# iiscleap/NeuralPlda

Measured on AMD Instinct MI355X. Metric: scored trial-pairs/sec (512-d xvec), higher is better.
Workload: dtype f32; 1 GPU; cfg1: 1048576 trial pairs/GPU/step, 512->150->150 NPLDA, scoring only (fused NeuralPlda.forward, inputs resident in HBM); xvector_dim=512, layer1_LDA_dim=150, layer2_PLDA_spkfactor_dim=150, params=kaldi-init truncated to 150, parallelism=trial-list shard x1, backend=single process, ranks_in_group=1

## Files before the change

### neuralplda_amd/csrc/nplda_fwd_dispatch.h

```cpp
#pragma once
#include <cstdlib>
#include <cstring>
#include "nplda_fwd_kernel.h"
#include "nplda_fwd_small.h"
#include "nplda_fwd_v2.h"
#include "nplda_fwd_v3.h"
#include "nplda_fwd_v5.h"
#include "nplda_fwd_v6.h"
#include "nplda_fwd_mid.h"

namespace nplda {

template <int MODE>
static inline int launch_fwd_v2(FwdArgs a, const NpldaLayout& L, hipStream_t st) {
    constexpr int WAVES = 8;
    const long long per_block = (MODE == MODE_EMBED ? 32 : 16) * WAVES;
    const long long blocks = (a.n + per_block - 1) / per_block;
    if (blocks > 0x7fffffffLL) return NPLDA_EINVAL;
    dim3 grid((unsigned)blocks), block(WAVES * 64);
#define NPLDA_LAUNCH(NBV) \
    hipLaunchKernelGGL((nplda_fwd_v2_kernel<NBV, MODE, WAVES, false, (NBV == 2 ? 4 : 2)>), grid, block, 0, st, a)
    switch (L.NB) {
        case 2: NPLDA_LAUNCH(2); break;
        case 4: NPLDA_LAUNCH(4); break;
        case 8: NPLDA_LAUNCH(8); break;
        case 10: NPLDA_LAUNCH(10); break;
        case 11: NPLDA_LAUNCH(11); break;
        case 12: NPLDA_LAUNCH(12); break;
        default: return NPLDA_EUNSUPPORTED;
    }
#undef NPLDA_LAUNCH
    return nplda_launch_status();
}

template <int MODE, int XM = 0>
static inline int launch_fwd_v3(FwdArgs a, const NpldaLayout& L, hipStream_t st) {
    constexpr int WAVES = 8;
    const long long per_block = (MODE == MODE_EMBED ? 32 : 16) * WAVES;
    const long long ntiles = (a.n + per_block - 1) / per_block;
    if (ntiles > 0x7fffffffLL) return NPLDA_EINVAL;
    int dev = 0, cus = 0;
    if (hipGetDevice(&dev) != hipSuccess ||
        hipDeviceGetAttribute(&cus, hipDeviceAttributeMultiprocessorCount, dev) != hipSuccess || cus <= 0)
        cus = 256;
    const long long blocks = ntiles < cus ? ntiles : cus;
    dim3 grid((unsigned)blocks), block(WAVES * 64);
#define NPLDA_LAUNCH(NBV) \
    hipLaunchKernelGGL((nplda_fwd_v3_kernel<NBV, MODE, WAVES, XM, (NBV == 2 ? 4 : 2)>), grid, block, 0, st, a, (int)ntiles)
    switch (L.NB) {
        case 2: NPLDA_LAUNCH(2); break;
        case 4: NPLDA_LAUNCH(4); break;
        case 8: NPLDA_LAUNCH(8); break;
        case 10: NPLDA_LAUNCH(10); break;
        default: return NPLDA_EUNSUPPORTED;
    }
#undef NPLDA_LAUNCH
    return nplda_launch_status();
}

template <int XM = 0>
static inline int launch_fwd_v5(FwdArgs a, const NpldaLayout& L, hipStream_t st) {
    constexpr int WAVES = 8;
    const long long ntiles = (a.n + 16 * WAVES - 1) / (16 * WAVES);
    if (ntiles > 0x7fffffffLL) return NPLDA_EINVAL;
    int dev = 0, cus = 0;
    if (hipGetDevice(&dev) != hipSuccess ||
        hipDeviceGetAttribute(&cus, hipDeviceAttributeMultiprocessorCount, dev) != hipSuccess || cus <= 0)
        cus = 256;
    const long long blocks = ntiles < cus ? ntiles : cus;
    dim3 grid((unsigned)blocks), block(WAVES * 64);
    switch (L.NB) {
        case 11: hipLaunchKernelGGL((nplda_fwd_v5_kernel<11, WAVES, 2, 6, 1, XM>), grid, block, 0, st, a, (int)ntiles); break;
        case 12: hipLaunchKernelGGL((nplda_fwd_v5_kernel<12, WAVES, 4, 4, 1, XM>), grid, block, 0, st, a, (int)ntiles); break;
        default: return NPLDA_EUNSUPPORTED;
    }
    return nplda_launch_status();
}

static inline bool fwd_v6_ok(const NpldaLayout& L) { return L.NB == 10 && L.D1 == 150 && L.D2 == 150; }
static inline bool fwd_v6_l2_f32() {
    static const bool f32 = getenv("NPLDA_FWD_V6_L2") != nullptr && strcmp(getenv("NPLDA_FWD_V6_L2"), "f32") == 0;
    return f32;
}
template <int XM = 0>
static inline int launch_fwd_v6(FwdArgs a, const NpldaLayout& L, hipStream_t st) {
    constexpr int WAVES = 8;
    const long long ntiles = (a.n + 16 * WAVES - 1) / (16 * WAVES);
    if (ntiles > 0x7fffffffLL) return NPLDA_EINVAL;
    if (!fwd_v6_ok(L)) return NPLDA_EUNSUPPORTED;
    int dev = 0, cus = 0;
    if (hipGetDevice(&dev) != hipSuccess ||
        hipDeviceGetAttribute(&cus, hipDeviceAttributeMultiprocessorCount, dev) != hipSuccess || cus <= 0)
        cus = 256;
    const long long blocks = ntiles < cus ? ntiles : cus;
    if (fwd_v6_l2_f32())
        hipLaunchKernelGGL((nplda_fwd_v6_kernel<10, 6, WAVES, 2, 5, 3, XM, 0, 2, 0>), dim3((unsigned)blocks), dim3(WAVES * 64), 0, st, a,
                           (int)ntiles);
    else
        hipLaunchKernelGGL((nplda_fwd_v6_kernel<10, 6, WAVES, 2, 5, 3, XM, 0, 2, 1>), dim3((unsigned)blocks), dim3(WAVES * 64), 0, st, a,
                           (int)ntiles);
    return nplda_launch_status();
}
template <int XM = 0>
static inline int launch_fwd_stream(FwdArgs a, const NpldaLayout& L, hipStream_t st) {
    static const bool no_v6 = getenv("NPLDA_FWD_NO_V6") != nullptr && getenv("NPLDA_FWD_NO_V6")[0] == '1';
    if (fwd_v6_ok(L) && !no_v6) return launch_fwd_v6<XM>(a, L, st);
    if (L.NB <= 10) return launch_fwd_v3<MODE_PAIR, XM>(a, L, st);
    return launch_fwd_v5<XM>(a, L, st);
}

template <int MODE>
static inline int launch_fwd_small(FwdArgs a, const NpldaLayout& L, hipStream_t st) {
    const long long per_block = (MODE == MODE_EMBED ? 32 : 16);
    const long long blocks = (a.n + per_block - 1) / per_block;
    dim3 grid((unsigned)blocks), block(256);
#define NPLDA_LAUNCH(NBV) hipLaunchKernelGGL((nplda_fwd_small_kernel<NBV, MODE>), grid, block, 0, st, a)
#define NPLDA_LAUNCH32(NBV)                                                                           \
    if (L.KS1 == 32 && L.D0 == 512) hipLaunchKernelGGL((nplda_fwd_small_kernel<NBV, MODE, 32>), grid, block, 0, st, a); \
    else NPLDA_LAUNCH(NBV)
    switch (L.NB) {
        case 2: NPLDA_LAUNCH(2); break;
        case 4: NPLDA_LAUNCH(4); break;
        case 8: NPLDA_LAUNCH(8); break;
        case 10: NPLDA_LAUNCH32(10); break;
        case 11: NPLDA_LAUNCH32(11); break;
        case 12: NPLDA_LAUNCH(12); break;
        default: return NPLDA_EUNSUPPORTED;
    }
#undef NPLDA_LAUNCH32
#undef NPLDA_LAUNCH
    return nplda_launch_status();
}

static inline int mid_cus() {
    int dev = 0, cus = 0;
    if (hipGetDevice(&dev) != hipSuccess ||
        hipDeviceGetAttribute(&cus, hipDeviceAttributeMultiprocessorCount, dev) != hipSuccess || cus <= 0)
        cus = 256;
    return cus;
}
template <bool EMBED = false>
static inline int launch_fwd_mid(FwdArgs a, const NpldaLayout& L, hipStream_t st) {
    const long long nh = EMBED ? (a.n + 15) / 16 : (a.n + 7) / 8;
    const int cus = mid_cus();
    long long grid = nh <= cus ? nh : ((nh + 1) / 2 < cus ? (nh + 1) / 2 : cus);
    if (grid < 1) grid = 1;
    const long long c = (nh + grid - 1) / grid;
    const long long r = nh - grid * (c - 1);
    if (c > 0x7fffffffLL) return NPLDA_EINVAL;
    const bool half = !(r == grid && (c & 1) == 0);
    const bool idx = a.ia != nullptr;
#define NPLDA_LAUNCH(NBV, HV, IV) \
    hipLaunchKernelGGL((nplda_fwd_mid_kernel<NBV, EMBED, HV, IV>), dim3((unsigned)grid), dim3(256), 0, st, a, (int)c, (int)r)
#define NPLDA_LAUNCH_H(NBV, HV) do { if (idx) { NPLDA_LAUNCH(NBV, HV, true); } else { NPLDA_LAUNCH(NBV, HV, false); } } while (0)
    switch (L.NB) {
        case 10: if (half) NPLDA_LAUNCH_H(10, true); else NPLDA_LAUNCH_H(10, false); break;
        case 11: if (half) NPLDA_LAUNCH_H(11, true); else NPLDA_LAUNCH_H(11, false); break;
        default: return NPLDA_EUNSUPPORTED;
    }
#undef NPLDA_LAUNCH_H
#undef NPLDA_LAUNCH
    return nplda_launch_status();
}

template <int MODE>
static inline int launch_fwd_old(FwdArgs a, const NpldaLayout& L, hipStream_t st) {
    a.D0 = L.D0; a.KS1 = L.KS1;
    a.oW2 = L.oW2; a.ob1 = L.ob1; a.ob2 = L.ob2; a.oQ = L.oQ; a.oP = L.oP; a.total = L.total;
    const long long units = (MODE == MODE_EMBED ? (a.n + 1) / 2 : a.n);
    if (units <= 256 * 64) return launch_fwd_small<MODE>(a, L, st);
    if constexpr (MODE == MODE_PAIR) return launch_fwd_stream<0>(a, L, st);
    return launch_fwd_v2<MODE>(a, L, st);
}

enum { FWD_SMALL = 0, FWD_MID = 1, FWD_STREAM = 2, FWD_SPLIT = 3 };
static inline long long pair_split_point(long long n, int cus) { return (n / 128 / cus) * 128 * cus; }
static inline int pair_kernel_choice(long long n, const NpldaLayout& L, int cus, long long* cost = nullptr, bool allow_split = true) {
    long long dummy;
    if (!cost) cost = &dummy;
    static const bool no_mid = getenv("NPLDA_FWD_NO_MID") != nullptr && getenv("NPLDA_FWD_NO_MID")[0] == '1';
    const bool mid_ok = !no_mid && (L.NB == 10 || L.NB == 11) && L.D0 == 512 && L.KS1 == 32;
    static const long long small_max = getenv("NPLDA_FWD_SMALL_MAX") ? atoll(getenv("NPLDA_FWD_SMALL_MAX")) : -1;
    const long long round_cost = L.NB == 10 ? 1000 : 1150;
    *cost = 120;
    if (mid_ok && small_max < 0 && n <= 8LL * cus) return FWD_MID;
    *cost = 190;
    if (n <= (small_max >= 0 ? small_max : 16LL * cus)) return FWD_SMALL;
    const long long rounds = ((n + 127) / 128 + cus - 1) / cus;
    const long long t_stream = 50 + rounds * round_cost;
    *cost = n <= 64LL * cus ? 190 * ((n + 16LL * cus - 1) / (16LL * cus)) : t_stream;
    if (!mid_ok) return n <= 64LL * cus ? FWD_SMALL : FWD_STREAM;
    const long long ch = ((n + 7) / 8 + cus - 1) / cus;
    const long long t_mid = 40 + (ch / 2) * (L.NB == 10 ? 133 : 168) + (ch & 1) * (L.NB == 10 ? 93 : 118);
    int best = t_mid < t_stream ? FWD_MID : FWD_STREAM;
    *cost = t_mid < t_stream ? t_mid : t_stream;
    static const bool no_split = getenv("NPLDA_FWD_NO_SPLIT") != nullptr && getenv("NPLDA_FWD_NO_SPLIT")[0] == '1';
    const long long full = pair_split_point(n, cus);
    if (allow_split && !no_split && full > 0 && full < n) {
        long long t_rem = 0;
        pair_kernel_choice(n - full, L, cus, &t_rem, false);
        const long long t_split = 50 + (full / 128 / cus) * round_cost + t_rem;
        if (t_split + 30 < *cost) {
            *cost = t_split;
            best = FWD_SPLIT;
        }
    }
    return best;
}

template <int MODE>
static inline int launch_fwd(FwdArgs a, const NpldaLayout& L, hipStream_t st) {
    if constexpr (MODE == MODE_PAIR) {
        const int cus = mid_cus();
        const int k = pair_kernel_choice(a.n, L, cus);
        a.D0 = L.D0; a.KS1 = L.KS1;
        a.oW2 = L.oW2; a.ob1 = L.ob1; a.ob2 = L.ob2; a.oQ = L.oQ; a.oP = L.oP; a.total = L.total;
        if (k == FWD_MID) return launch_fwd_mid<false>(a, L, st);
        if (k == FWD_SMALL) return launch_fwd_small<MODE>(a, L, st);
        if (k == FWD_SPLIT && a.ia == nullptr && a.ib == nullptr) {
            const long long full = pair_split_point(a.n, cus);
            FwdArgs b = a;
            b.xa += full * a.ldx; b.xb += full * a.ldx; b.out_s += full; b.n = a.n - full;
            a.n = full;
            if (int rc = launch_fwd_stream<0>(a, L, st)) return rc;
            const int kr = pair_kernel_choice(b.n, L, cus, nullptr, false);
            if (kr == FWD_MID) return launch_fwd_mid<false>(b, L, st);
            if (kr == FWD_SMALL) return launch_fwd_small<MODE>(b, L, st);
            return launch_fwd_stream<0>(b, L, st);
        }
        return launch_fwd_stream<0>(a, L, st);
    }
    if constexpr (MODE == MODE_EMBED) {
        if (a.out_y == nullptr && pair_kernel_choice((a.n + 1) / 2, L, mid_cus(), nullptr, false) == FWD_MID) {
            a.D0 = L.D0; a.KS1 = L.KS1;
            a.oW2 = L.oW2; a.ob1 = L.ob1; a.ob2 = L.ob2; a.oQ = L.oQ; a.oP = L.oP; a.total = L.total;
            return launch_fwd_mid<true>(a, L, st);
        }
    }
    return launch_fwd_old<MODE>(a, L, st);
}

static inline int launch_fwd_pairs_bf16rows(FwdArgs a, const NpldaLayout& L, hipStream_t st) {
    const int k = pair_kernel_choice(a.n, L, mid_cus());
    if (k != FWD_STREAM && k != FWD_SPLIT) return NPLDA_EUNSUPPORTED;
    a.D0 = L.D0; a.KS1 = L.KS1;
    a.oW2 = L.oW2; a.ob1 = L.ob1; a.ob2 = L.ob2; a.oQ = L.oQ; a.oP = L.oP; a.total = L.total;
    return launch_fwd_stream<2>(a, L, st);
}

static inline const char* pair_kernel_name(long long n, const NpldaLayout& L) {
    switch (pair_kernel_choice(n, L, mid_cus())) {
        case FWD_SPLIT:
            return pair_kernel_name(pair_split_point(n, mid_cus()), L);
        case FWD_SMALL: return "nplda_fwd_small_kernel (4 waves share a 16-pair tile, feature-split)";
        case FWD_MID: return "nplda_fwd_mid_kernel (balanced 16-pair tiles, K-split layer 1, groups of 2 tiles)";
        default:
            if (fwd_v6_ok(L) && !(getenv("NPLDA_FWD_NO_V6") != nullptr && getenv("NPLDA_FWD_NO_V6")[0] == '1'))
                return fwd_v6_l2_f32()
                           ? "nplda_fwd_v6_kernel (persistent, 9 feature blocks on 16x16x4 MFMAs + 6 features on 4x4x1 MFMAs)"
                           : "nplda_fwd_v6_kernel (persistent, layer 1: 9 feature blocks on 16x16x4 MFMAs + 6 features on 4x4x1 "
                             "MFMAs; layer 2: split bf16x3, 6 passes of 16x16x32)";
            return L.NB <= 10 ? "nplda_fwd_v3_kernel (persistent, 8 waves x 16 pairs, weights through LDS)"
                              : "nplda_fwd_v5_kernel (persistent, LDS-DMA weight chunks, layer 2 by output groups)";
    }
}

static inline int check_model(int D0, int D1, int D2) {
    if (D0 <= 0 || D1 <= 0 || D2 <= 0 || (D0 % 4) != 0) return NPLDA_EINVAL;
    if (!nplda_dims_ok(D0, D1, D2)) return NPLDA_EUNSUPPORTED;
    return NPLDA_OK;
}

static inline bool rows_ok(const float* x, int64_t ld, int D) {
    return x && ld >= D && (ld % 4) == 0 && nplda_aligned16(x);
}

}
```

Baseline: 366.2 million pairs/s.

## Add hybrid v6h kernel running part of layer 1 on split-bf16x3 MFMAs

Adds a new persistent kernel in which layer 1 computes some 16-wide feature blocks with fp32 16x16x4 MFMAs and S1 blocks with weights and inputs split into three bf16 parts, using 16x16x32 bf16 MFMAs. The split W1 blocks are converted by register staging into LDS alongside the existing DMA path. This replaces the old 4x4x1 MFMA handling of the leftover features. Dispatch uses it by default with S1=3, selectable through environment variables. The aim is to move more layer-1 work onto higher-throughput bf16 MFMAs while keeping near-fp32 accuracy, at the cost of extra split ALU work, more LDS, and register pressure.

After: 383.4 million pairs/s (median of 6 runs). 1.05x the previous value.

```diff
diff --git a/neuralplda_amd/csrc/nplda_fwd_dispatch.h b/neuralplda_amd/csrc/nplda_fwd_dispatch.h
--- a/neuralplda_amd/csrc/nplda_fwd_dispatch.h
+++ b/neuralplda_amd/csrc/nplda_fwd_dispatch.h
@@ -7,6 +7,7 @@
 #include "nplda_fwd_v3.h"
 #include "nplda_fwd_v5.h"
 #include "nplda_fwd_v6.h"
+#include "nplda_fwd_v6h.h"
 #include "nplda_fwd_mid.h"
 
 namespace nplda {
@@ -82,6 +83,22 @@
     static const bool f32 = getenv("NPLDA_FWD_V6_L2") != nullptr && strcmp(getenv("NPLDA_FWD_V6_L2"), "f32") == 0;
     return f32;
 }
+enum { FWD_V6H_S1_DEFAULT = 3 };
+static inline bool fwd_v6h_s1_built(int s1) { return s1 == 2 || s1 == 3 || s1 == 4; }
+static inline int fwd_v6h_s1_env() {
+    static const int s1 = [] {
+        const char* f = getenv("NPLDA_FWD_V6_L1");
+        if (f != nullptr && strcmp(f, "f32") == 0) return 0;
+        const char* n = getenv("NPLDA_FWD_V6_L1S");
+        if (n != nullptr && fwd_v6h_s1_built(atoi(n))) return atoi(n);
+        return (int)FWD_V6H_S1_DEFAULT;
+    }();
+    return s1;
+}
+static inline int fwd_v6h_s1(const NpldaLayout& L) {
+    if (!fwd_v6_ok(L) || fwd_v6_l2_f32() || (L.KS1 & 1) != 0) return 0;
+    return fwd_v6h_s1_env();
+}
 template <int XM = 0>
 static inline int launch_fwd_v6(FwdArgs a, const NpldaLayout& L, hipStream_t st) {
     constexpr int WAVES = 8;
@@ -93,12 +110,17 @@
         hipDeviceGetAttribute(&cus, hipDeviceAttributeMultiprocessorCount, dev) != hipSuccess || cus <= 0)
         cus = 256;
     const long long blocks = ntiles < cus ? ntiles : cus;
-    if (fwd_v6_l2_f32())
-        hipLaunchKernelGGL((nplda_fwd_v6_kernel<10, 6, WAVES, 2, 5, 3, XM, 0, 2, 0>), dim3((unsigned)blocks), dim3(WAVES * 64), 0, st, a,
-                           (int)ntiles);
-    else
-        hipLaunchKernelGGL((nplda_fwd_v6_kernel<10, 6, WAVES, 2, 5, 3, XM, 0, 2, 1>), dim3((unsigned)blocks), dim3(WAVES * 64), 0, st, a,
-                           (int)ntiles);
+    const dim3 grid((unsigned)blocks), block(WAVES * 64);
+    switch (fwd_v6h_s1(L)) {
+        case 2: hipLaunchKernelGGL((nplda_fwd_v6h_kernel<10, WAVES, 2, 4, XM>), grid, block, 0, st, a, (int)ntiles); break;
+        case 3: hipLaunchKernelGGL((nplda_fwd_v6h_kernel<10, WAVES, 3, 4, XM>), grid, block, 0, st, a, (int)ntiles); break;
+        case 4: hipLaunchKernelGGL((nplda_fwd_v6h_kernel<10, WAVES, 4, 3, XM>), grid, block, 0, st, a, (int)ntiles); break;
+        default:
+            if (fwd_v6_l2_f32())
+                hipLaunchKernelGGL((nplda_fwd_v6_kernel<10, 6, WAVES, 2, 5, 3, XM, 0, 2, 0>), grid, block, 0, st, a, (int)ntiles);
+            else
+                hipLaunchKernelGGL((nplda_fwd_v6_kernel<10, 6, WAVES, 2, 5, 3, XM, 0, 2, 1>), grid, block, 0, st, a, (int)ntiles);
+    }
     return nplda_launch_status();
 }
 template <int XM = 0>
@@ -255,11 +277,22 @@
         case FWD_SMALL: return "nplda_fwd_small_kernel (4 waves share a 16-pair tile, feature-split)";
         case FWD_MID: return "nplda_fwd_mid_kernel (balanced 16-pair tiles, K-split layer 1, groups of 2 tiles)";
         default:
-            if (fwd_v6_ok(L) && !(getenv("NPLDA_FWD_NO_V6") != nullptr && getenv("NPLDA_FWD_NO_V6")[0] == '1'))
+            if (fwd_v6_ok(L) && !(getenv("NPLDA_FWD_NO_V6") != nullptr && getenv("NPLDA_FWD_NO_V6")[0] == '1')) {
+                switch (fwd_v6h_s1(L)) {
+#define NPLDA_V6H_LABEL(S1, NF)                                                                                            \
+    "nplda_fwd_v6_kernel (persistent, hybrid layer 1 = nplda_fwd_v6h_kernel, S1 = " #S1 ": " #NF " feature blocks on 16x16x4 " \
+    "MFMAs + " #S1 " blocks split bf16x3; layer 2: split bf16x3, 6 passes of 16x16x32)"
+                    case 2: return NPLDA_V6H_LABEL(2, 8);
+                    case 3: return NPLDA_V6H_LABEL(3, 7);
+                    case 4: return NPLDA_V6H_LABEL(4, 6);
+#undef NPLDA_V6H_LABEL
+                    default: break;
+                }
                 return fwd_v6_l2_f32()
                            ? "nplda_fwd_v6_kernel (persistent, 9 feature blocks on 16x16x4 MFMAs + 6 features on 4x4x1 MFMAs)"
                            : "nplda_fwd_v6_kernel (persistent, layer 1: 9 feature blocks on 16x16x4 MFMAs + 6 features on 4x4x1 "
                              "MFMAs; layer 2: split bf16x3, 6 passes of 16x16x32)";
+            }
             return L.NB <= 10 ? "nplda_fwd_v3_kernel (persistent, 8 waves x 16 pairs, weights through LDS)"
                               : "nplda_fwd_v5_kernel (persistent, LDS-DMA weight chunks, layer 2 by output groups)";
     }
diff --git a/neuralplda_amd/csrc/nplda_fwd_v6h.h b/neuralplda_amd/csrc/nplda_fwd_v6h.h
--- /dev/null
+++ b/neuralplda_amd/csrc/nplda_fwd_v6h.h
@@ -0,0 +1,345 @@
+#pragma once
+#include "nplda_fwd_kernel.h"
+#include "nplda_fwd_bf16x3.h"
+
+namespace nplda {
+
+template <int N>
+__device__ __forceinline__ void mfma6_blocks(const WFrag (&w)[N], const bf16x8 ah, const bf16x8 am, const bf16x8 al,
+                                             const bf16x8 bh, const bf16x8 bm, const bf16x8 bl, f32x4* accA, f32x4* accB) {
+#define NPLDA_PASS(P, XA, XB)                                  \
+    _Pragma("unroll") for (int u = 0; u < N; ++u) {            \
+        accA[u] = NPLDA_MFMA_BF16(w[u].P, XA, accA[u]);        \
+        accB[u] = NPLDA_MFMA_BF16(w[u].P, XB, accB[u]);        \
+    }
+    NPLDA_PASS(m, am, bm)
+    NPLDA_PASS(h, al, bl)
+    NPLDA_PASS(l, ah, bh)
+    NPLDA_PASS(h, am, bm)
+    NPLDA_PASS(m, ah, bh)
+    NPLDA_PASS(h, ah, bh)
+#undef NPLDA_PASS
+}
+
+template <int NB, int WAVES, int S1, int G1, int XM = 0>
+__global__ __launch_bounds__(WAVES * 64, WAVES / 4) void nplda_fwd_v6h_kernel(const FwdArgs a, int ntiles) {
+    constexpr int KPB = 2;
+    constexpr int NF = NB - S1;
+    constexpr int STEP4 = NB * 64;
+    constexpr int CH1 = STEP4 * KPB;
+    constexpr int NSEG1 = NF * KPB;
+    constexpr int NGR = (NF + G1 - 1) / G1;
+    constexpr int KC2 = NB / 2;
+    constexpr int SG = S1 % 2 ? 3 : 2;
+    static_assert(S1 >= 1 && S1 <= WAVES && S1 < NB && (S1 % 2 == 0 || S1 >= 3), "one W1 unit per wave at the most");
+    static_assert((WAVES & (WAVES - 1)) == 0, "the owner of a W1 unit is computed mod WAVES");
+    static_assert(NB % 2 == 0 && WAVES <= NB && NB <= 2 * WAVES, "split layer 2: k32-steps of two whole accumulator blocks, one "
+                                                                 "or two W2 units per wave");
+    __shared__ f32x4 wbuf[2][CH1];
+    __shared__ bf16x8 wsp1[2][S1 * 3 * 64];
+    __shared__ bf16x8 wsp[2][NB * 3 * 64];
+    __shared__ f32x4 cvec[4][NB * 4];
+    __shared__ f32x4 sink[64];
+
+    const int tid = threadIdx.x;
+    const int lane = tid & 63;
+    const int wave = __builtin_amdgcn_readfirstlane(tid >> 6);
+    const int j = lane & 15;
+    const int g = lane >> 4;
+
+    const f32x4* Wall = reinterpret_cast<const f32x4*>(a.packed);
+    const long long w2base4 = (long long)(a.oW2 / 4);
+    for (int i = tid; i < 4 * NB * 4; i += WAVES * 64) {
+        const int v = i / (NB * 4), e = i % (NB * 4);
+        const size_t o = v == 0 ? a.ob1 : (v == 1 ? a.ob2 : (v == 2 ? a.oQ : a.oP));
+        cvec[v][e] = reinterpret_cast<const f32x4*>(a.packed + o)[e];
+    }
+    const f32x4* b1p = cvec[0];
+    const f32x4* b2p = cvec[1];
+    const f32x4* Qp = cvec[2];
+    const f32x4* Pp = cvec[3];
+    const int D0 = a.D0;
+    const int NC1 = a.KS1 / KPB;
+
+    auto seg_dma = [&](const f32x4* src, f32x4* dst) {
+        unsigned lo = (unsigned)lane * 16u;
+        asm volatile("" : "+v"(lo));
+        __builtin_amdgcn_global_load_lds((const __attribute__((address_space(1))) void*)(reinterpret_cast<const char*>(src) + lo),
+                                         (__attribute__((address_space(3))) void*)dst, 16, 0, 0);
+    };
+    auto dma_l1 = [&](int c, f32x4* dst) {
+        const f32x4* src = Wall + (long long)c * CH1;
+#pragma unroll
+        for (int i = 0; i < (NSEG1 + WAVES - 1) / WAVES; ++i) {
+            const int sgm = wave + WAVES * i;
+            const bool live = sgm < NSEG1;
+            const int sg = live ? sgm : 0;
+            const int off = (sg / NF) * STEP4 + (sg % NF) * 64;
+            seg_dma(src + off, live ? dst + off : sink);
+        }
+    };
+    auto chunk_fence = [&]() {
+        __builtin_amdgcn_s_waitcnt(0x0070);
+        __builtin_amdgcn_s_barrier();
+        __builtin_amdgcn_sched_barrier(0);
+    };
+    f32x4 w1lo, w1hi;
+    auto w1_unit = [&](int cn) { return (wave - cn * S1) & (WAVES - 1); };
+    auto w1_load = [&](int cn) {
+        const int u = w1_unit(cn);
+        const char* base = reinterpret_cast<const char*>(Wall + (long long)(2 * cn) * STEP4 + (NF + (u < S1 ? u : 0)) * 64);
+        unsigned lo = (unsigned)lane * 16u;
+        asm volatile("" : "+v"(lo));
+        w1lo = *reinterpret_cast<const f32x4*>(base + lo);
+        w1hi = *reinterpret_cast<const f32x4*>(base + STEP4 * 16 + lo);
+    };
+    auto w1_store = [&](int cn, bf16x8* dst) {
+        const int u = w1_unit(cn);
+        if (u < S1) {
+            bf16x8 h, m, l;
+            split3x8(w1lo, w1hi, h, m, l);
+            dst[(u * 3 + 0) * 64 + lane] = h;
+            dst[(u * 3 + 1) * 64 + lane] = m;
+            dst[(u * 3 + 2) * 64 + lane] = l;
+        }
+    };
+    f32x4 w2lo[2], w2hi[2];
+    const bool two = wave + WAVES < NB;
+    auto w2_load = [&](int c, int i, int r) {
+        const int nb = wave + WAVES * i;
+        const char* base = reinterpret_cast<const char*>(Wall + w2base4 + (long long)(2 * c) * STEP4 + (nb < NB ? nb : 0) * 64);
+        unsigned lo = (unsigned)lane * 16u;
+        asm volatile("" : "+v"(lo));
+        w2lo[r] = *reinterpret_cast<const f32x4*>(base + lo);
+        w2hi[r] = *reinterpret_cast<const f32x4*>(base + STEP4 * 16 + lo);
+    };
+    auto w2_store = [&](int i, int r, bf16x8* dst) {
+        const int nb = wave + WAVES * i;
+        bf16x8 h, m, l;
+        split3x8(w2lo[r], w2hi[r], h, m, l);
+        dst[(nb * 3 + 0) * 64 + lane] = h;
+        dst[(nb * 3 + 1) * 64 + lane] = m;
+        dst[(nb * 3 + 2) * 64 + lane] = l;
+    };
+
+    auto tile_ptrs = [&](long long t, long long& t0, bool& ok, const float*& pa, const float*& pb) {
+        t0 = (t * WAVES + wave) * 16;
+        long long r = t0 + j;
+        ok = r < a.n;
+        if (!ok) r = a.n - 1;
+        pa = x_row<XM>(a.xa, r, a.ldx);
+        pb = x_row<XM>(a.xb, r, a.ldx);
+    };
+    long long tile = blockIdx.x;
+    long long t0;
+    bool ok;
+    const float *sa, *sb;
+    tile_ptrs(tile, t0, ok, sa, sb);
+
+    const int cn1 = NC1 > 1 ? 1 : 0;
+    dma_l1(0, wbuf[0]);
+    w1_load(0);
+    f32x4 xa[KPB], xb[KPB];
+#pragma unroll
+    for (int s = 0; s < KPB; ++s) {
+        xa[s] = load_xrow<XM>(sa, 16 * s + 4 * g, D0);
+        xb[s] = load_xrow<XM>(sb, 16 * s + 4 * g, D0);
+    }
+    w1_store(0, wsp1[0]);
+    w1_load(cn1);
+    __syncthreads();
+    chunk_fence();
+    int par = 0;
+
+    for (;;) {
+        const long long tile_n = tile + gridDim.x;
+
+        f32x4 accA[NB], accB[NB];
+#pragma unroll
+        for (int nb = 0; nb < NB; ++nb) {
+            accA[nb] = b1p[4 * nb + g];
+            accB[nb] = accA[nb];
+        }
+
+        auto chunk = [&](int c, f32x4 (&xc)[KPB], f32x4 (&yc)[KPB], f32x4 (&xn)[KPB], f32x4 (&yn)[KPB]) {
+            const bool more = (c + 1 < NC1);
+            if (more) {
+                w1_store(c + 1, wsp1[par ^ 1]);
+                dma_l1(c + 1, wbuf[par ^ 1]);
+                if (c + 2 < NC1) w1_load(c + 2);
+            } else {
+                w2_load(0, 0, 0);
+                w2_load(0, 1, 1);
+            }
+#pragma unroll
+            for (int s = 0; s < KPB; ++s) {
+                const int ks = more ? KPB * (c + 1) + s : KPB * c + s;
+                xn[s] = load_xrow<XM>(sa, 16 * ks + 4 * g, D0);
+                yn[s] = load_xrow<XM>(sb, 16 * ks + 4 * g, D0);
+            }
+            __builtin_amdgcn_sched_barrier(0);
+            const f32x4* w = wbuf[par];
+            const bf16x8* wp = wsp1[par];
+            bf16x8 ah, am, al, bh, bm, bl;
+            split3x8(xc[0], xc[1], ah, am, al);
+            split3x8(yc[0], yc[1], bh, bm, bl);
+            auto fp32_step = [&](int s) {
+#pragma unroll
+                for (int gr = 0; gr < NGR; ++gr) {
+                    const int nb0 = gr * G1;
+                    f32x4 av[G1];
+#pragma unroll
+                    for (int u = 0; u < G1; ++u)
+                        if (nb0 + u < NF) av[u] = w[s * STEP4 + (nb0 + u) * 64 + lane];
+#pragma unroll
+                    for (int r = 0; r < 4; ++r) {
+#pragma unroll
+                        for (int u = 0; u < G1; ++u) {
+                            if (nb0 + u < NF) {
+                                accA[nb0 + u] = __builtin_amdgcn_mfma_f32_16x16x4f32(av[u][r], xc[s][r], accA[nb0 + u], 0, 0, 0);
+                                accB[nb0 + u] = __builtin_amdgcn_mfma_f32_16x16x4f32(av[u][r], yc[s][r], accB[nb0 + u], 0, 0, 0);
+                            }
+                        }
+                    }
+                }
+            };
+            fp32_step(0);
+            {
+                WFrag wf[SG];
+#pragma unroll
+                for (int u = 0; u < SG; ++u) {
+                    wf[u].h = wp[(u * 3 + 0) * 64 + lane];
+                    wf[u].m = wp[(u * 3 + 1) * 64 + lane];
+                    wf[u].l = wp[(u * 3 + 2) * 64 + lane];
+                }
+                mfma6_blocks<SG>(wf, ah, am, al, bh, bm, bl, &accA[NF], &accB[NF]);
+            }
+#pragma unroll
+            for (int u0 = SG; u0 < S1; u0 += 2) {
+                WFrag wf[2];
+#pragma unroll
+                for (int u = 0; u < 2; ++u) {
+                    wf[u].h = wp[((u0 + u) * 3 + 0) * 64 + lane];
+                    wf[u].m = wp[((u0 + u) * 3 + 1) * 64 + lane];
+                    wf[u].l = wp[((u0 + u) * 3 + 2) * 64 + lane];
+                }
+                mfma6_blocks<2>(wf, ah, am, al, bh, bm, bl, &accA[NF + u0], &accB[NF + u0]);
+            }
+            fp32_step(1);
+            if (!more) {
+                w2_store(0, 0, wsp[0]);
+                if (two) w2_store(1, 1, wsp[0]);
+            }
+            chunk_fence();
+            par ^= 1;
+        };
+        f32x4 xan[KPB], xbn[KPB];
+        int c = 0;
+        for (; c + 1 < NC1; c += 2) {
+            chunk(c, xa, xb, xan, xbn);
+            chunk(c + 1, xan, xbn, xa, xb);
+        }
+        if (c < NC1) {
+            chunk(c, xa, xb, xan, xbn);
+#pragma unroll
+            for (int s = 0; s < KPB; ++s) {
+                xa[s] = xan[s];
+                xb[s] = xbn[s];
+            }
+        }
+
+        {
+            float ssA = 0.f, ssB = 0.f;
+#pragma unroll
+            for (int nb = 0; nb < NB; ++nb) {
+#pragma unroll
+                for (int r = 0; r < 4; ++r) {
+                    ssA = fmaf(accA[nb][r], accA[nb][r], ssA);
+                    ssB = fmaf(accB[nb][r], accB[nb][r], ssB);
+                }
+            }
+            ssA = wave_xor_add(ssA, 16); ssA = wave_xor_add(ssA, 32);
+            ssB = wave_xor_add(ssB, 16); ssB = wave_xor_add(ssB, 32);
+            const float invA = 1.0f / fmaxf(sqrtf(ssA), 1e-12f);
+            const float invB = 1.0f / fmaxf(sqrtf(ssB), 1e-12f);
+#pragma unroll
+            for (int nb = 0; nb < NB; ++nb) {
+                accA[nb] *= invA;
+                accB[nb] *= invB;
+            }
+        }
+
+        float part = 0.f;
+        f32x4 zA[NB], zB[NB];
+#pragma unroll
+        for (int nb = 0; nb < NB; ++nb) {
+            zA[nb] = b2p[4 * nb + g];
+            zB[nb] = zA[nb];
+        }
+#pragma unroll
+        for (int c2 = 0; c2 < KC2; ++c2) {
+            const bool more = c2 + 1 < KC2;
+            if (more) {
+                w2_load(c2 + 1, 0, 0);
+            } else {
+                dma_l1(0, wbuf[par]);
+                w1_load(0);
+                long long t0_x;
+                bool ok_x;
+                const float *pa, *pb;
+                tile_ptrs(tile_n, t0_x, ok_x, pa, pb);
+#pragma unroll
+                for (int s = 0; s < KPB; ++s) {
+                    xa[s] = load_xrow<XM>(pa, 16 * s + 4 * g, D0);
+                    xb[s] = load_xrow<XM>(pb, 16 * s + 4 * g, D0);
+                }
+            }
+            bf16x8 ah, am, al, bh, bm, bl;
+            split3x8(accA[2 * c2], accA[2 * c2 + 1], ah, am, al);
+            split3x8(accB[2 * c2], accB[2 * c2 + 1], bh, bm, bl);
+            const bf16x8* w = wsp[c2 & 1];
+#pragma unroll
+            for (int nb = 0; nb < NB; nb += 2) {
+                WFrag w0, w1;
+                w0.h = w[(nb * 3 + 0) * 64 + lane];
+                w0.m = w[(nb * 3 + 1) * 64 + lane];
+                w0.l = w[(nb * 3 + 2) * 64 + lane];
+                w1.h = w[(nb * 3 + 3) * 64 + lane];
+                w1.m = w[(nb * 3 + 4) * 64 + lane];
+                w1.l = w[(nb * 3 + 5) * 64 + lane];
+                mfma6x4(w0, w1, ah, am, al, bh, bm, bl, zA[nb], zB[nb], zA[nb + 1], zB[nb + 1]);
+                if (nb == 2 * ((NB / 2) / 2)) {
+                    if (more) {
+                        w2_store(0, 0, wsp[(c2 + 1) & 1]);
+                        w2_load(c2 + 1, 1, 0);
+                    } else {
+                        w1_store(0, wsp1[par]);
+                        w1_load(cn1);
+                    }
+                }
+            }
+            if (more && two) w2_store(1, 0, wsp[(c2 + 1) & 1]);
+            chunk_fence();
+        }
+#pragma unroll
+        for (int nb = 0; nb < NB; ++nb) {
+            const f32x4 q = Qp[4 * nb + g];
+            const f32x4 p = Pp[4 * nb + g];
+#pragma unroll
+            for (int r = 0; r < 4; ++r) {
+                const float z1 = zA[nb][r], z2 = zB[nb][r];
+                part = fmaf(q[r], fmaf(z1, z1, z2 * z2), part);
+                part = fmaf(2.0f * p[r], z1 * z2, part);
+            }
+        }
+        part = wave_xor_add(part, 16);
+        part = wave_xor_add(part, 32);
+        if (g == 0 && ok) a.out_s[t0 + j] = part;
+
+        tile = tile_n;
+        if (tile >= ntiles) break;
+        tile_ptrs(tile, t0, ok, sa, sb);
+    }
+}
+
+}
```
